# Windere/EAS-SNN

Measured on AMD Instinct MI355X. Metric: event-frames/sec (T=3) SYOLOX-S Gen1 304x240, higher is better.
Workload: dtype f32

## Files before the change

### eas_snn_amd/csrc/bn_lif.hip

```cpp
#include <stdlib.h>

#include <string.h>

#include "bn_lif_policy.h"
#include "eas_common.h"

namespace {

constexpr int VEC = 4;
constexpr int kMaxChunks = 64;
constexpr int NW = EAS_BLOCK / EAS_WAVE;

static inline int pick_chunks(int64_t groups_per_channel, int C) {
    int64_t want = (groups_per_channel + EAS_BLOCK - 1) / EAS_BLOCK;
    int64_t cap = 8192 / (C > 0 ? C : 1);
    if (cap < 1) cap = 1;
    if (cap > kMaxChunks) cap = kMaxChunks;
    if (want > cap) want = cap;
    if (want < 1) want = 1;
    return (int)want;
}

__global__ __launch_bounds__(EAS_BLOCK) void bn_stats_partial(const float* __restrict__ y, int TN, int C, int HW,
                                                              double* __restrict__ part, int Cy) {
// ... 4 lines not shown
    double s = 0.0, ss = 0.0;
    const int64_t stride = (int64_t)gridDim.x * blockDim.x;
    GroupWalk gw((int64_t)blockIdx.x * blockDim.x + threadIdx.x, stride, hw4);
    int64_t g = (int64_t)blockIdx.x * blockDim.x + threadIdx.x;
    for (; g + stride < groups; g += 2 * stride) {
        const float4 v0 = reinterpret_cast<const float4*>(y + (((int64_t)gw.n * Cy + c) * (int64_t)HW))[gw.q];
        gw.next();
        const float4 v1 = reinterpret_cast<const float4*>(y + (((int64_t)gw.n * Cy + c) * (int64_t)HW))[gw.q];
        gw.next();
        s += (double)v0.x + (double)v0.y + (double)v0.z + (double)v0.w;
        ss += (double)v0.x * v0.x + (double)v0.y * v0.y + (double)v0.z * v0.z + (double)v0.w * v0.w;
        s += (double)v1.x + (double)v1.y + (double)v1.z + (double)v1.w;
        ss += (double)v1.x * v1.x + (double)v1.y * v1.y + (double)v1.z * v1.z + (double)v1.w * v1.w;
    }
    if (g < groups) {
        const float4 v = reinterpret_cast<const float4*>(y + (((int64_t)gw.n * Cy + c) * (int64_t)HW))[gw.q];
        s += (double)v.x + (double)v.y + (double)v.z + (double)v.w;
        ss += (double)v.x * v.x + (double)v.y * v.y + (double)v.z * v.z + (double)v.w * v.w;
    }
    const double ts = eas_block_sum<double, NW>(s, red);
    const double tss = eas_block_sum<double, NW>(ss, red);
    if (threadIdx.x == 0) {
        part[((int64_t)c * kMaxChunks + blockIdx.x) * 2 + 0] = ts;
        part[((int64_t)c * kMaxChunks + blockIdx.x) * 2 + 1] = tss;
    }
}

__global__ __launch_bounds__(EAS_BLOCK) void bn_stats_partial_scalar(const float* __restrict__ y, int TN, int C, int HW,
                                                                     double* __restrict__ part) {
    __shared__ double red[NW];
    const int c = blockIdx.y;
    const int64_t groups = (int64_t)TN * HW;
    double s = 0.0, ss = 0.0;
    for (int64_t g = (int64_t)blockIdx.x * blockDim.x + threadIdx.x; g < groups; g += (int64_t)gridDim.x * blockDim.x) {
        const int64_t n = g / HW;
        const int q = (int)(g - n * HW);
        const float v = y[(n * C + c) * (int64_t)HW + q];
        s += v;
        ss += (double)v * v;
    }
    const double ts = eas_block_sum<double, NW>(s, red);
    const double tss = eas_block_sum<double, NW>(ss, red);
    if (threadIdx.x == 0) {
        part[((int64_t)c * kMaxChunks + blockIdx.x) * 2 + 0] = ts;
        part[((int64_t)c * kMaxChunks + blockIdx.x) * 2 + 1] = tss;
    }
}

__global__ __launch_bounds__(EAS_WAVE) void bn_stats_finalize(const double* __restrict__ part, int nchunks, double count,
                                                              int replicas, float eps, float momentum, float* __restrict__ mean,
                                                              float* __restrict__ invstd, float* __restrict__ rmean,
                                                              float* __restrict__ rvar) {
    const int c = blockIdx.x;
    double s = 0.0, ss = 0.0;
    if ((int)threadIdx.x < nchunks) {
        s = part[((int64_t)c * kMaxChunks + threadIdx.x) * 2 + 0];
        ss = part[((int64_t)c * kMaxChunks + threadIdx.x) * 2 + 1];
    }
    s = eas_wave_sum(s);
    ss = eas_wave_sum(ss);
    if (threadIdx.x == 0) {
        const double m = s / count;
        double var = ss / count - m * m;
        if (var < 0.0) var = 0.0;
        mean[c] = (float)m;
        invstd[c] = (float)(1.0 / sqrt(var + (double)eps));
        if (rmean) {
            const double full = count * replicas;
            const double unbiased = full > 1.0 ? var * full / (full - 1.0) : var;
            rmean[c] = (float)((1.0 - momentum) * rmean[c] + momentum * m);
            rvar[c] = (float)((1.0 - momentum) * rvar[c] + momentum * unbiased);
        }
    }
}

struct BnLifOut {
    const float* residual;
    int out_ctot;
    int y_ctot;
};

typedef __bf16 bf16x8 __attribute__((ext_vector_type(8)));

template <int T_, bool HARD, bool DI, bool STRICT>
__global__ __launch_bounds__(EAS_BLOCK) void bn_lif_fwd_kernel(const float* __restrict__ y, const float* __restrict__ mean,
                                                               const float* __restrict__ invstd,
                                                               const float* __restrict__ gamma,
                                                               const float* __restrict__ beta, const float* v_in, float* v_out,
                                                               EasLifParams p, float* __restrict__ spikes,
                                                               float* __restrict__ mean_out, int N, int C, int HW, int bcast,
                                                               BnFin fin, BnLifOut ox) {
    __shared__ float st[2];
    const int c = blockIdx.z * 8 + blockIdx.x;
    if (c >= C) return;
    const int chunk = blockIdx.y, nchunks_g = gridDim.y;
    float mu, istd;
    if (fin.part) {
        bn_finalize_in_block(fin, c, st, mu, istd, chunk == 0);
    } else {
        mu = mean[c];
        istd = invstd[c];
    }
    const float scale = gamma[c] * istd;
    const float shift = beta[c] - mu * scale;
    const int64_t Mo = ox.out_ctot ? (int64_t)N * ox.out_ctot * HW : (int64_t)N * C * HW;
    const float k = eas_lif_k(p);
    const float omk = 1.0f - k;
    const int hw4 = HW / VEC;
    const int64_t groups = (int64_t)N * hw4;
    const int64_t M = (int64_t)N * C * HW;
    const int Cy = ox.y_ctot ? ox.y_ctot : C;
    const int64_t yts = bcast ? 0 : (int64_t)N * Cy * HW;
    GroupWalk gw((int64_t)chunk * blockDim.x + threadIdx.x, (int64_t)nchunks_g * blockDim.x, hw4);
    for (int64_t g = (int64_t)chunk * blockDim.x + threadIdx.x; g < groups; g += (int64_t)nchunks_g * blockDim.x, gw.next()) {
        const int64_t n = gw.n;
        const int q = gw.q;
        const int64_t base = (n * C + c) * (int64_t)HW + (int64_t)q * VEC;
        float4 ys[T_];
        const int64_t ybase = (n * Cy + c) * (int64_t)HW + (int64_t)q * VEC;
#pragma unroll
        for (int t = 0; t < T_; ++t) ys[t] = *reinterpret_cast<const float4*>(y + (int64_t)t * yts + ybase);
        const float vr0 = HARD ? p.v_reset : 0.0f;
        float4 v = v_in ? *reinterpret_cast<const float4*>(v_in + base) : make_float4(vr0, vr0, vr0, vr0);
        float4 acc = make_float4(0.f, 0.f, 0.f, 0.f);
#pragma unroll
        for (int t = 0; t < T_; ++t) {
            float4 h, s;
            eas_lif_step<HARD, DI, STRICT>(v.x, fmaf(ys[t].x, scale, shift), k, omk, p.v_th, p.v_reset, h.x, s.x);
            eas_lif_step<HARD, DI, STRICT>(v.y, fmaf(ys[t].y, scale, shift), k, omk, p.v_th, p.v_reset, h.y, s.y);
            eas_lif_step<HARD, DI, STRICT>(v.z, fmaf(ys[t].z, scale, shift), k, omk, p.v_th, p.v_reset, h.z, s.z);
            eas_lif_step<HARD, DI, STRICT>(v.w, fmaf(ys[t].w, scale, shift), k, omk, p.v_th, p.v_reset, h.w, s.w);
            acc.x += s.x; acc.y += s.y; acc.z += s.z; acc.w += s.w;
            if (ox.residual) {
                const float4 r = *reinterpret_cast<const float4*>(ox.residual + (int64_t)t * M + base);
                s.x += r.x; s.y += r.y; s.z += r.z; s.w += r.w;
            }
            const int64_t obase = ox.out_ctot ? (n * ox.out_ctot + c) * (int64_t)HW + (int64_t)q * VEC : base;
            *reinterpret_cast<float4*>(spikes + (int64_t)t * Mo + obase) = s;
        }
        if (v_out) *reinterpret_cast<float4*>(v_out + base) = v;
        if (mean_out) {
            const float Tf = (float)T_;
            *reinterpret_cast<float4*>(mean_out + base) = make_float4(acc.x / Tf, acc.y / Tf, acc.z / Tf, acc.w / Tf);
        }
    }
}

__global__ __launch_bounds__(EAS_BLOCK) void bn_finalize_kernel(BnFin fin) {
    __shared__ float st[2];
    float mu, istd;
    bn_finalize_in_block(fin, (int)blockIdx.x, st, mu, istd, true);
}

template <int T_, bool HARD, bool DI, bool STRICT, int PV>
__global__ __launch_bounds__(EAS_BLOCK) void bn_lif_fwd_sp_kernel(const float* __restrict__ y, const float* __restrict__ mean,
                                                                  const float* __restrict__ invstd, const float* __restrict__ gamma,
                                                                  const float* __restrict__ beta, const float* v_in, float* v_out,
                                                                  EasLifParams p, bf16x8* __restrict__ planes, const bf16x8* __restrict__ res_planes,
                                                                  float* __restrict__ mean_out, int N, int C, int HW, int bcast, int y_ctot,
                                                                  int out_groups_tot, int res_groups_tot) {
    typedef float vecp __attribute__((ext_vector_type(PV)));
    const int grp = blockIdx.z * 8 + blockIdx.x;
    const int G = C / 8;
    if (grp >= G) return;
    const int chunk = blockIdx.y, nchunks_g = gridDim.y;
    float scale[8], shift[8];
#pragma unroll
    for (int j = 0; j < 8; ++j) {
        const int c = 8 * grp + j;
        scale[j] = gamma[c] * invstd[c];
        shift[j] = beta[c] - mean[c] * scale[j];
    }
    const float k = eas_lif_k(p);
    const float omk = 1.0f - k;
    const int hwp = HW / PV;
    const int64_t groups = (int64_t)N * hwp;
    const int Cy = y_ctot ? y_ctot : C;
    const int64_t yts = bcast ? 0 : (int64_t)N * Cy * HW;
    const float vr0 = HARD ? p.v_reset : 0.0f;
    const float Tf = (float)T_;
    GroupWalk gw((int64_t)chunk * blockDim.x + threadIdx.x, (int64_t)nchunks_g * blockDim.x, hwp);
    for (int64_t g = (int64_t)chunk * blockDim.x + threadIdx.x; g < groups; g += (int64_t)nchunks_g * blockDim.x, gw.next()) {
        const int64_t n = gw.n;
        const int q = gw.q;
        vecp ys[8][T_];
#pragma unroll
        for (int j = 0; j < 8; ++j) {
            const int64_t yb = (n * Cy + 8 * grp + j) * (int64_t)HW + (int64_t)q * PV;
#pragma unroll
            for (int t = 0; t < T_; ++t) ys[j][t] = *reinterpret_cast<const vecp*>(y + (int64_t)t * yts + yb);
        }
        float v[8][PV], acc[8][PV];
#pragma unroll
        for (int j = 0; j < 8; ++j) {
            vecp v0;
            if (v_in) v0 = *reinterpret_cast<const vecp*>(v_in + (n * C + 8 * grp + j) * (int64_t)HW + (int64_t)q * PV);
#pragma unroll
            for (int e = 0; e < PV; ++e) { v[j][e] = v_in ? v0[e] : vr0; acc[j][e] = 0.f; }
        }
#pragma unroll
        for (int t = 0; t < T_; ++t) {
            bf16x8 rp[PV];
            if (res_planes) {
#pragma unroll
                for (int e = 0; e < PV; ++e) rp[e] = res_planes[(((int64_t)t * N + n) * res_groups_tot + grp) * (int64_t)HW + (int64_t)q * PV + e];
            }
#pragma unroll
            for (int e = 0; e < PV; ++e) {
                bf16x8 o;
#pragma unroll
                for (int j = 0; j < 8; ++j) {
                    float h, s;
                    eas_lif_step<HARD, DI, STRICT>(v[j][e], fmaf(ys[j][t][e], scale[j], shift[j]), k, omk, p.v_th, p.v_reset, h, s);
                    acc[j][e] += s;
                    if (res_planes) s += (float)rp[e][j];
                    o[j] = (__bf16)s;
                }
                planes[(((int64_t)t * N + n) * out_groups_tot + grp) * (int64_t)HW + (int64_t)q * PV + e] = o;
            }
        }
#pragma unroll
        for (int j = 0; j < 8; ++j) {
            const int64_t base = (n * C + 8 * grp + j) * (int64_t)HW + (int64_t)q * PV;
            if (v_out) {
                vecp o;
#pragma unroll
                for (int e = 0; e < PV; ++e) o[e] = v[j][e];
                *reinterpret_cast<vecp*>(v_out + base) = o;
            }
            if (mean_out) {
                vecp o;
#pragma unroll
                for (int e = 0; e < PV; ++e) o[e] = acc[j][e] / Tf;
                *reinterpret_cast<vecp*>(mean_out + base) = o;
            }
        }
    }
}

template <int T_, bool HARD, bool DI, bool STRICT, class POL>
__device__ __forceinline__ void recompute_dz(const float (&yv)[T_], const float (&gs)[T_], float v0, float scale,
                                             float shift, float k, float omk, const EasLifParams& p, bool detach,
                                             int sg_id, float alpha, float (&dz)[T_], float& dk, float& da) {
    float h[T_], vprev[T_], z[T_];
    float v = v0;
#pragma unroll
    for (int t = 0; t < T_; ++t) {
        float s;
        vprev[t] = v;
        z[t] = fmaf(yv[t], scale, shift);
        eas_lif_step<HARD, DI, STRICT>(v, z[t], k, omk, p.v_th, p.v_reset, h[t], s);
    }
    float gv = 0.f;
#pragma unroll
    for (int t = T_ - 1; t >= 0; --t) {
        float dkt, gx;
        if constexpr (POL::fast)
            eas_lif_step_bwd_ct<HARD, DI, STRICT, POL::sg, POL::detach>(gs[t], gv, h[t], vprev[t], z[t], k, omk, p.v_th, p.v_reset, alpha, dkt,
                                                                        gx, da);
        else
            eas_lif_step_bwd<HARD, DI, STRICT>(gs[t], gv, h[t], vprev[t], z[t], k, omk, p.v_th, p.v_reset, detach, sg_id, alpha, dkt, gx, da);
        dz[t] = gx;
        dk += dkt;
    }
}

template <int T_, bool HARD, bool DI, bool STRICT, bool APPLY, class POL>
__global__ __launch_bounds__(EAS_BLOCK) void bn_lif_bwd_kernel(
    const float* __restrict__ grad_s, const float* __restrict__ grad_mean, const float* __restrict__ y,
    const float* __restrict__ mean, const float* __restrict__ invstd, const float* __restrict__ gamma,
    const float* __restrict__ beta, const float* __restrict__ v_init, EasLifParams p, int sg_id, float alpha,
    int batch_stats, double* __restrict__ part, int nchunks, float* __restrict__ grad_y, float* __restrict__ grad_gamma,
    float* __restrict__ grad_beta, float* __restrict__ grad_w, int N, int C, int HW, int bcast, int gs_ctot, int y_ctot,
    const float* __restrict__ alpha_dev, float* __restrict__ grad_alpha, int c_begin, int c_end, int finalize) {
    __shared__ double red[NW];
    __shared__ float bc[2];
    constexpr bool FAST = POL::fast;
    if (FAST) { bcast = 0; sg_id = POL::sg; }
    if (alpha_dev) alpha = fabsf(*alpha_dev);
    const int c = c_begin + blockIdx.z * 8 + blockIdx.x;
    if (c >= c_end) return;
    const int chunk = blockIdx.y, nchunks_g = gridDim.y;
    const float mu = mean[c], istd = invstd[c];
    const float scale = gamma[c] * istd;
    const float shift = beta[c] - mu * scale;
    const float k = eas_lif_k(p);
    const float omk = 1.0f - k;
    const bool detach = (p.flags & EAS_LIF_DETACH_RESET) != 0;
    const int hw4 = HW / VEC;
    const int64_t groups = (int64_t)N * hw4;
    const int64_t M = (int64_t)N * C * HW;
    const float invT = 1.0f / (float)T_;
    const int Cy = y_ctot ? y_ctot : C;
    const int64_t My = (int64_t)N * Cy * HW;
    const int64_t yts = bcast ? 0 : My;
    const int64_t Mg = gs_ctot ? (int64_t)N * gs_ctot * HW : M;
    const int Cg = gs_ctot ? gs_ctot : C;
    float m1 = 0.f, m2 = 0.f;
    if (APPLY) {
        if (threadIdx.x < EAS_WAVE) {
            double s1 = 0.0, s2 = 0.0;
            if ((int)threadIdx.x < nchunks) {
                s1 = part[((int64_t)c * kMaxChunks + threadIdx.x) * 4 + 0];
                s2 = part[((int64_t)c * kMaxChunks + threadIdx.x) * 4 + 1];
            }
            s1 = eas_wave_sum(s1);
            s2 = eas_wave_sum(s2);
            if (threadIdx.x == 0) {
                const double cnt = (double)T_ * N * HW;
                bc[0] = (float)(s1 / cnt);
                bc[1] = (float)(s2 / cnt);
                if (chunk == 0) {
                    grad_beta[c] = (float)s1;
                    grad_gamma[c] = (float)s2;
                }
            }
        }
        __syncthreads();
        if (batch_stats) { m1 = bc[0]; m2 = bc[1]; }
    }
    float s1 = 0.f, s2 = 0.f, dk = 0.f, da = 0.f;
    GroupWalk gw((int64_t)chunk * blockDim.x + threadIdx.x, (int64_t)nchunks_g * blockDim.x, hw4);
    for (int64_t g = (int64_t)chunk * blockDim.x + threadIdx.x; g < groups; g += (int64_t)nchunks_g * blockDim.x, gw.next()) {
        const int64_t n = gw.n;
        const int q = gw.q;
        const int64_t base = (n * C + c) * (int64_t)HW + (int64_t)q * VEC;
        float4 ys[T_], gsv[T_];
        const int64_t ybase = (n * Cy + c) * (int64_t)HW + (int64_t)q * VEC;
#pragma unroll
        for (int t = 0; t < T_; ++t) ys[t] = *reinterpret_cast<const float4*>(y + (int64_t)t * yts + ybase);
        float4 gm = make_float4(0.f, 0.f, 0.f, 0.f);
        if (!FAST && grad_mean) {
            gm = *reinterpret_cast<const float4*>(grad_mean + base);
            gm.x *= invT; gm.y *= invT; gm.z *= invT; gm.w *= invT;
        }
#pragma unroll
        for (int t = 0; t < T_; ++t) {
            gsv[t] = gm;
            if (FAST || grad_s) {
                const int64_t gbase = FAST ? (n * Cg + c) * (int64_t)HW + (int64_t)q * VEC
                                           : (gs_ctot ? (n * gs_ctot + c) * (int64_t)HW + (int64_t)q * VEC : base);
                const float4 g4 = *reinterpret_cast<const float4*>(grad_s + (int64_t)t * Mg + gbase);
                gsv[t].x += g4.x; gsv[t].y += g4.y; gsv[t].z += g4.z; gsv[t].w += g4.w;
            }
        }
        const float vr0 = HARD ? p.v_reset : 0.0f;
        float4 v0 = make_float4(vr0, vr0, vr0, vr0);
        if (!FAST && v_init) v0 = *reinterpret_cast<const float4*>(v_init + base);
        float4 outv[T_];
#pragma unroll
        for (int e = 0; e < VEC; ++e) {
            float yv[T_], gs[T_], dz[T_];
#pragma unroll
            for (int t = 0; t < T_; ++t) {
                yv[t] = reinterpret_cast<const float*>(&ys[t])[e];
                gs[t] = reinterpret_cast<const float*>(&gsv[t])[e];
            }
            const float v0e = reinterpret_cast<const float*>(&v0)[e];
            float dke = 0.f;
            recompute_dz<T_, HARD, DI, STRICT, POL>(yv, gs, v0e, scale, shift, k, omk, p, detach, sg_id, alpha, dz, dke, da);
#pragma unroll
            for (int t = 0; t < T_; ++t) {
                const float xhat = (yv[t] - mu) * istd;
                if (APPLY) {
                    reinterpret_cast<float*>(&outv[t])[e] = scale * (dz[t] - m1 - xhat * m2);
                } else {
                    s1 += dz[t];
                    s2 += dz[t] * xhat;
                }
            }
            dk += dke;
        }
        if (APPLY) {
            if (bcast) {
                float4 a = outv[0];
#pragma unroll
                for (int t = 1; t < T_; ++t) { a.x += outv[t].x; a.y += outv[t].y; a.z += outv[t].z; a.w += outv[t].w; }
                *reinterpret_cast<float4*>(grad_y + ybase) = a;
            } else {
#pragma unroll
                for (int t = 0; t < T_; ++t) *reinterpret_cast<float4*>(grad_y + (int64_t)t * My + ybase) = outv[t];
            }
        }
    }
    if (APPLY && grad_w && finalize && chunk == 0 && c == c_begin) {
        double acc = 0.0;
        for (int i = threadIdx.x; i < C * nchunks; i += blockDim.x) {
            const int cc = i / nchunks, j = i - cc * nchunks;
            acc += part[((int64_t)cc * kMaxChunks + j) * 4 + 2];
        }
        const double tot = eas_block_sum<double, NW>(acc, red);
        if (threadIdx.x == 0) *grad_w = (float)tot * (k * (1.0f - k));
    }
    if (APPLY && grad_alpha && finalize && chunk == 0 && c == c_begin) {
        double acc = 0.0;
        for (int i = threadIdx.x; i < C * nchunks; i += blockDim.x) {
            const int cc = i / nchunks, j = i - cc * nchunks;
            acc += part[((int64_t)cc * kMaxChunks + j) * 4 + 3];
        }
        const double tot = eas_block_sum<double, NW>(acc, red);
        if (threadIdx.x == 0) {
            const float a = *alpha_dev;
            *grad_alpha = (float)tot * (a > 0.f ? 1.f : (a < 0.f ? -1.f : 0.f));
        }
    }
    if (!APPLY) {
        const double t1 = eas_block_sum<double, NW>((double)s1, red);
        const double t2 = eas_block_sum<double, NW>((double)s2, red);
        const double t3 = eas_block_sum<double, NW>((double)dk, red);
        double t4 = 0.0;
        if (sg_id == EAS_SG_PATAN) t4 = eas_block_sum<double, NW>((double)da, red);
        if (threadIdx.x == 0) {
            double* o = part + ((int64_t)c * kMaxChunks + chunk) * 4;
            o[0] = t1; o[1] = t2; o[2] = t3; o[3] = t4;
        }
    }
}

template <int T_, bool HARD, bool DI, bool STRICT, int NT_, int GPT, class POL>
__global__ __launch_bounds__(NT_) void bn_lif_bwd_small_kernel(
    const float* __restrict__ grad_s, const float* __restrict__ grad_mean, const float* __restrict__ y,
    const float* __restrict__ mean, const float* __restrict__ invstd, const float* __restrict__ gamma,
    const float* __restrict__ beta, const float* __restrict__ v_init, EasLifParams p, int sg_id, float alpha,
    int batch_stats, double* __restrict__ part, float* __restrict__ grad_y, float* __restrict__ grad_gamma,
    float* __restrict__ grad_beta, int N, int C, int HW, int gs_ctot, int y_ctot, const float* __restrict__ alpha_dev) {
    constexpr int NWV = NT_ / EAS_WAVE;
    __shared__ double red[4][NWV];
    __shared__ float bc[2];
    if (POL::fast) sg_id = POL::sg;
    if (alpha_dev) alpha = fabsf(*alpha_dev);
    const int c = blockIdx.x;
    const float mu = mean[c], istd = invstd[c];
    const float scale = gamma[c] * istd;
    const float shift = beta[c] - mu * scale;
    const float k = eas_lif_k(p);
    const float omk = 1.0f - k;
    const bool detach = (p.flags & EAS_LIF_DETACH_RESET) != 0;
    const int hw4 = HW / VEC;
    const int groups = N * hw4;
    const int64_t M = (int64_t)N * C * HW;
    const int Cy = y_ctot ? y_ctot : C;
    const int64_t My = (int64_t)N * Cy * HW;
    const int64_t Mg = gs_ctot ? (int64_t)N * gs_ctot * HW : M;
    const float invT = 1.0f / (float)T_;
    float4 ys[GPT][T_], gsv[GPT][T_], v0[GPT];
    int64_t ybase[GPT];
#pragma unroll
    for (int i = 0; i < GPT; ++i) {
        const int g = threadIdx.x + i * NT_;
        const int gg = g < groups ? g : groups - 1;
        const int n = gg / hw4, q = gg - n * hw4;
        const int64_t base = ((int64_t)n * C + c) * (int64_t)HW + (int64_t)q * VEC;
        ybase[i] = ((int64_t)n * Cy + c) * (int64_t)HW + (int64_t)q * VEC;
#pragma unroll
        for (int t = 0; t < T_; ++t) ys[i][t] = *reinterpret_cast<const float4*>(y + (int64_t)t * My + ybase[i]);
        float4 gm = make_float4(0.f, 0.f, 0.f, 0.f);
        if (grad_mean) {
            gm = *reinterpret_cast<const float4*>(grad_mean + base);
            gm.x *= invT; gm.y *= invT; gm.z *= invT; gm.w *= invT;
        }
#pragma unroll
        for (int t = 0; t < T_; ++t) {
            gsv[i][t] = gm;
            if (grad_s) {
                const int64_t gbase = gs_ctot ? ((int64_t)n * gs_ctot + c) * (int64_t)HW + (int64_t)q * VEC : base;
                const float4 g4 = *reinterpret_cast<const float4*>(grad_s + (int64_t)t * Mg + gbase);
                gsv[i][t].x += g4.x; gsv[i][t].y += g4.y; gsv[i][t].z += g4.z; gsv[i][t].w += g4.w;
            }
        }
        const float vr0 = HARD ? p.v_reset : 0.0f;
        v0[i] = make_float4(vr0, vr0, vr0, vr0);
        if (v_init) v0[i] = *reinterpret_cast<const float4*>(v_init + base);
    }
    float s1 = 0.f, s2 = 0.f, dk = 0.f, da = 0.f;
#pragma unroll
    for (int i = 0; i < GPT; ++i) {
        const bool live = threadIdx.x + i * NT_ < groups;
#pragma unroll
        for (int e = 0; e < VEC; ++e) {
            float yv[T_], gs[T_], dz[T_];
#pragma unroll
            for (int t = 0; t < T_; ++t) {
                yv[t] = reinterpret_cast<const float*>(&ys[i][t])[e];
                gs[t] = reinterpret_cast<const float*>(&gsv[i][t])[e];
            }
            float dke = 0.f, dae = 0.f;
            recompute_dz<T_, HARD, DI, STRICT, POL>(yv, gs, reinterpret_cast<const float*>(&v0[i])[e], scale, shift, k, omk, p, detach, sg_id, alpha, dz, dke, dae);
            if (live) {
#pragma unroll
                for (int t = 0; t < T_; ++t) {
                    s1 += dz[t];
                    s2 += dz[t] * ((yv[t] - mu) * istd);
                }
                dk += dke;
                da += dae;
            }
        }
    }
    double t1 = eas_wave_sum((double)s1), t2 = eas_wave_sum((double)s2), t3 = eas_wave_sum((double)dk), t4 = eas_wave_sum((double)da);
    if ((threadIdx.x & (EAS_WAVE - 1)) == 0) {
        const int w = threadIdx.x / EAS_WAVE;
        red[0][w] = t1; red[1][w] = t2; red[2][w] = t3; red[3][w] = t4;
    }
    __syncthreads();
    if (threadIdx.x == 0) {
        t1 = t2 = t3 = t4 = 0.0;
        for (int w = 0; w < NWV; ++w) { t1 += red[0][w]; t2 += red[1][w]; t3 += red[2][w]; t4 += red[3][w]; }
        const double cnt = (double)T_ * N * HW;
        bc[0] = (float)(t1 / cnt);
        bc[1] = (float)(t2 / cnt);
        grad_beta[c] = (float)t1;
        grad_gamma[c] = (float)t2;
        double* o = part + ((int64_t)c * kMaxChunks) * 4;
        o[0] = t1; o[1] = t2; o[2] = t3; o[3] = sg_id == EAS_SG_PATAN ? t4 : 0.0;
    }
    __syncthreads();
    const float m1 = batch_stats ? bc[0] : 0.f, m2 = batch_stats ? bc[1] : 0.f;
#pragma unroll
    for (int i = 0; i < GPT; ++i) {
        if (threadIdx.x + i * NT_ >= groups) continue;
        float4 outv[T_];
#pragma unroll
        for (int e = 0; e < VEC; ++e) {
            float yv[T_], gs[T_], dz[T_];
#pragma unroll
            for (int t = 0; t < T_; ++t) {
                yv[t] = reinterpret_cast<const float*>(&ys[i][t])[e];
                gs[t] = reinterpret_cast<const float*>(&gsv[i][t])[e];
            }
            float dke = 0.f, dae = 0.f;
            recompute_dz<T_, HARD, DI, STRICT, POL>(yv, gs, reinterpret_cast<const float*>(&v0[i])[e], scale, shift, k, omk, p, detach, sg_id, alpha, dz, dke, dae);
#pragma unroll
            for (int t = 0; t < T_; ++t) reinterpret_cast<float*>(&outv[t])[e] = scale * (dz[t] - m1 - ((yv[t] - mu) * istd) * m2);
        }
#pragma unroll
        for (int t = 0; t < T_; ++t) *reinterpret_cast<float4*>(grad_y + (int64_t)t * My + ybase[i]) = outv[t];
    }
}

__global__ __launch_bounds__(EAS_BLOCK) void bn_lif_bwd_scalars_kernel(const double* __restrict__ part, int C, EasLifParams p, float* __restrict__ grad_w,
                                                                       const float* __restrict__ alpha_dev, float* __restrict__ grad_alpha) {
    __shared__ double red[NW];
    const float k = eas_lif_k(p);
    if (grad_w) {
        double acc = 0.0;
        for (int i = threadIdx.x; i < C; i += blockDim.x) acc += part[((int64_t)i * kMaxChunks) * 4 + 2];
        const double tot = eas_block_sum<double, NW>(acc, red);
        if (threadIdx.x == 0) *grad_w = (float)tot * (k * (1.0f - k));
    }
    if (grad_alpha) {
        double acc = 0.0;
        for (int i = threadIdx.x; i < C; i += blockDim.x) acc += part[((int64_t)i * kMaxChunks) * 4 + 3];
        const double tot = eas_block_sum<double, NW>(acc, red);
        if (threadIdx.x == 0) {
            const float a = *alpha_dev;
            *grad_alpha = (float)tot * (a > 0.f ? 1.f : (a < 0.f ? -1.f : 0.f));
        }
    }
}

template <int T_, bool HARD, bool DI, bool STRICT>
int launch_fwd_t(const float* y, const float* mean, const float* invstd, const float* gamma, const float* beta,
                 const float* v_in, float* v_out, EasLifParams p, float* spikes, float* mean_out, int N, int C, int HW,
                 int bcast, const BnFin& fin, const BnLifOut& ox, bf16x8* planes, const bf16x8* res_planes, int out_groups, int res_groups,
                 hipStream_t st) {
    if (planes) {
        if (fin.part) {
            EAS_LAUNCH(bn_finalize_kernel, dim3(C), dim3(EAS_BLOCK), 0, st, fin);
            EAS_CHECK_LAUNCH();
        }
        constexpr int PV = 1;
        const int chunks = pick_chunks((int64_t)N * (HW / PV), C / 8);
        EAS_LAUNCH((bn_lif_fwd_sp_kernel<T_, HARD, DI, STRICT, PV>), EAS_CHAN_GRID(chunks, C / 8), dim3(EAS_BLOCK), 0, st, y,
                           mean, invstd, gamma, beta, v_in,
                           v_out, p, planes, res_planes, mean_out, N, C, HW, bcast, ox.y_ctot, out_groups, res_groups);
        EAS_CHECK_LAUNCH();
        return EAS_OK;
    }
    const int chunks = pick_chunks((int64_t)N * (HW / VEC), C);
    EAS_LAUNCH((bn_lif_fwd_kernel<T_, HARD, DI, STRICT>), EAS_CHAN_GRID(chunks, C), dim3(EAS_BLOCK), 0, st, y, mean,
                       invstd, gamma, beta, v_in, v_out, p, spikes, mean_out, N, C, HW, bcast, fin, ox);
    EAS_CHECK_LAUNCH();
    return EAS_OK;
}

template <bool HARD, bool DI, bool STRICT>
int launch_fwd(int T, const float* y, const float* mean, const float* invstd, const float* gamma, const float* beta,
               const float* v_in, float* v_out, EasLifParams p, float* spikes, float* mean_out, int N, int C, int HW,
               int bcast, const BnFin& fin, const BnLifOut& ox, bf16x8* planes, const bf16x8* res_planes, int out_groups, int res_groups,
               hipStream_t st) {
#define EAS_CASE(TT) \
    case TT: return launch_fwd_t<TT, HARD, DI, STRICT>(y, mean, invstd, gamma, beta, v_in, v_out, p, spikes, mean_out, N, C, HW, bcast, fin, ox, planes, res_planes, out_groups, res_groups, st);
    switch (T) {
        EAS_CASE(1) EAS_CASE(2) EAS_CASE(3) EAS_CASE(4) EAS_CASE(5) EAS_CASE(6) EAS_CASE(7) EAS_CASE(8)
        default: return EAS_ERR_UNSUPPORTED;
    }
#undef EAS_CASE
}

struct BwdCall {
    const float *grad_s, *grad_mean, *y, *mean, *invstd, *gamma, *beta, *v_init;
    EasLifParams p;
    int sg;
    float alpha;
    int batch_stats;
    float *grad_y, *grad_gamma, *grad_beta, *grad_w;
    double* ws;
    int T, N, C, HW, bcast, gs_ctot, y_ctot;
    const float* alpha_dev;
    float* grad_alpha;
    hipStream_t st;
};

static inline bool bwd_form(const char* word) {
    const char* form = getenv("EAS_BNLIF_BWD");
    return form && strstr(form, word);
}

static inline int bwd_one_pass_gpt(const BwdCall& c) {
    const int gpt = c.T <= 3 ? 3 : (c.T <= 5 ? 2 : 1);
    const int64_t groups = (int64_t)c.N * (c.HW / VEC);
    return (!bwd_form("two") && !c.bcast && c.C >= 64 && groups <= 512 * gpt) ? gpt : 0;
}

template <int T_, bool HARD, bool DI, bool STRICT, class POL>
int launch_bwd_t(const BwdCall& c) {
    const int N = c.N, C = c.C, HW = c.HW;
    const int chunks = pick_chunks((int64_t)N * (HW / VEC), C);
    if (bwd_one_pass_gpt(c)) {
        constexpr int GPT = T_ <= 3 ? 3 : (T_ <= 5 ? 2 : 1);
        const int64_t groups = (int64_t)N * (HW / VEC);
#define EAS_SMALL(NT_) EAS_LAUNCH((bn_lif_bwd_small_kernel<T_, HARD, DI, STRICT, NT_, GPT, POL>), dim3(C), dim3(NT_), 0, c.st, c.grad_s, c.grad_mean, c.y, \
                                   c.mean, c.invstd, c.gamma, c.beta, c.v_init, c.p, c.sg, c.alpha, c.batch_stats, c.ws, c.grad_y, c.grad_gamma,       \
                                   c.grad_beta, N, C, HW, c.gs_ctot, c.y_ctot, c.alpha_dev)
        if (groups <= 256 * GPT) EAS_SMALL(256);
        else EAS_SMALL(512);
#undef EAS_SMALL
        EAS_CHECK_LAUNCH();
        if (c.grad_w || c.grad_alpha) {
            EAS_LAUNCH(bn_lif_bwd_scalars_kernel, dim3(1), dim3(EAS_BLOCK), 0, c.st, c.ws, C, c.p, c.grad_w, c.alpha_dev, c.grad_alpha);
            EAS_CHECK_LAUNCH();
        }
        return EAS_OK;
    }
    static const int group_mb = eas_dev_env("EAS_BNLIF_BWD_GROUP_MB") ? atoi(eas_dev_env("EAS_BNLIF_BWD_GROUP_MB")) : 0;
    int gc = C;
    if (group_mb > 0) {
        const double per_channel = (double)N * HW * 4.0 * ((c.bcast ? 1 : T_) + T_);
        gc = (int)(group_mb * 1048576.0 / per_channel) / 8 * 8;
        if (gc < 8) gc = 8;
        if (gc > C) gc = C;
    }
    for (int c0 = 0; c0 < C; c0 += gc) {
        const int c1 = c0 + gc < C ? c0 + gc : C;
        const int last = c1 == C;
        EAS_LAUNCH((bn_lif_bwd_kernel<T_, HARD, DI, STRICT, false, POL>), EAS_CHAN_GRID(chunks, c1 - c0), dim3(EAS_BLOCK), 0, c.st, c.grad_s,
                   c.grad_mean, c.y, c.mean, c.invstd, c.gamma, c.beta, c.v_init, c.p, c.sg, c.alpha, c.batch_stats, c.ws, chunks, c.grad_y,
                   c.grad_gamma, c.grad_beta, (float*)nullptr, N, C, HW, c.bcast, c.gs_ctot, c.y_ctot, c.alpha_dev, (float*)nullptr, c0, c1, 0);
        EAS_CHECK_LAUNCH();
        EAS_LAUNCH((bn_lif_bwd_kernel<T_, HARD, DI, STRICT, true, POL>), EAS_CHAN_GRID(chunks, c1 - c0), dim3(EAS_BLOCK), 0, c.st, c.grad_s,
                   c.grad_mean, c.y, c.mean, c.invstd, c.gamma, c.beta, c.v_init, c.p, c.sg, c.alpha, c.batch_stats, c.ws, chunks, c.grad_y,
                   c.grad_gamma, c.grad_beta, c.grad_w, N, C, HW, c.bcast, c.gs_ctot, c.y_ctot, c.alpha_dev, c.grad_alpha, c0, c1, last);
        EAS_CHECK_LAUNCH();
    }
    return EAS_OK;
}

struct BwdRow {
    int T;
    bool hard, di;
    int sg;
    bool detach;
    int (*fn)(const BwdCall&);
};
template <int T_, bool HARD, bool DI, int SG = EAS_SG_RUNTIME, bool DETACH = false>
constexpr BwdRow bwd_row() {
    return {T_, HARD, DI, SG, DETACH, launch_bwd_t<T_, HARD, DI, false, BnLifBwdPolicy<SG, DETACH>>};
}
#define EAS_BWD_GENERIC_ROWS(H, D) \
    bwd_row<1, H, D>(), bwd_row<2, H, D>(), bwd_row<3, H, D>(), bwd_row<4, H, D>(), bwd_row<5, H, D>(), bwd_row<6, H, D>(), bwd_row<7, H, D>(), bwd_row<8, H, D>()
const BwdRow kBwdInstances[] = {
    bwd_row<3, false, false, EAS_SG_ATAN>(), bwd_row<5, false, false, EAS_SG_ATAN>(), bwd_row<7, false, false, EAS_SG_ATAN>(),
    EAS_BWD_GENERIC_ROWS(false, false), EAS_BWD_GENERIC_ROWS(true, false), EAS_BWD_GENERIC_ROWS(false, true), EAS_BWD_GENERIC_ROWS(true, true),
};
#undef EAS_BWD_GENERIC_ROWS

int bwd_select(const BwdCall& c) {
    const bool hard = c.p.flags & EAS_LIF_HARD_RESET, di = c.p.flags & EAS_LIF_DECAY_INPUT, detach = c.p.flags & EAS_LIF_DETACH_RESET;
    if (c.p.flags & EAS_LIF_FIRE_STRICT) return EAS_ERR_UNSUPPORTED;
    const bool plain = bwd_one_pass_gpt(c) || (c.grad_s && !c.grad_mean && !c.v_init && !c.bcast);
    const bool fast_ok = plain && !bwd_form("generic");
    for (const BwdRow& r : kBwdInstances) {
        if (r.T != c.T || r.hard != hard || r.di != di) continue;
        if (r.sg == EAS_SG_RUNTIME || (fast_ok && r.sg == c.sg && r.detach == detach)) return r.fn(c);
    }
    return EAS_ERR_UNSUPPORTED;
}

}

extern "C" {

int64_t eas_bn_workspace_doubles(int C) { return (int64_t)C * kMaxChunks * 4; }

static int stats_partial(const float* y, int TN, int C, int HW, double* workspace, int y_ctot, hipStream_t st) {
    const int Cy = y_ctot ? y_ctot : C;
    int chunks;
    if (HW % VEC == 0 && (((uintptr_t)y) & 15) == 0) {
        chunks = pick_chunks((int64_t)TN * (HW / VEC), C);
        EAS_LAUNCH(bn_stats_partial, dim3(chunks, C), dim3(EAS_BLOCK), 0, st, y, TN, C, HW, workspace, Cy);
    } else {
        if (Cy != C) return EAS_ERR_UNSUPPORTED;
        chunks = pick_chunks((int64_t)TN * HW, C);
        EAS_LAUNCH(bn_stats_partial_scalar, dim3(chunks, C), dim3(EAS_BLOCK), 0, st, y, TN, C, HW, workspace);
    }
    if (hipGetLastError() != hipSuccess) return EAS_ERR_LAUNCH;
    return chunks;
}

int eas_bn_stats(const float* y, int TN, int C, int HW, int replicas, float eps, float momentum, float* mean,
                 float* invstd, float* running_mean, float* running_var, double* workspace, eas_stream_t stream) {
    if (!y || !mean || !invstd || !workspace || TN < 1 || C < 1 || HW < 1 || replicas < 1) return EAS_ERR_INVALID_ARG;
    if ((running_mean == nullptr) != (running_var == nullptr)) return EAS_ERR_INVALID_ARG;
    if (C > 65535) return EAS_ERR_UNSUPPORTED;
    hipStream_t st = eas_s(stream);
    EAS_CLEAR_ERR();
    const int chunks = stats_partial(y, TN, C, HW, workspace, 0, st);
    if (chunks < 0) return chunks;
// ... 126 lines not shown
```

### eas_snn_amd/csrc/eas_common.h

```cpp
#pragma once
#include <hip/hip_runtime.h>
#include <stdint.h>
#include <stdlib.h>

#include "../../include/eas_hip.h"

#define EAS_WAVE 64
#define EAS_BLOCK 256

#define EAS_CLEAR_ERR() (void)hipGetLastError()
#define EAS_CHECK_LAUNCH()                                          \
    do {                                                            \
        if (hipGetLastError() != hipSuccess) return EAS_ERR_LAUNCH; \
    } while (0)

static inline hipStream_t eas_s(eas_stream_t s) { return reinterpret_cast<hipStream_t>(s); }

__attribute__((visibility("hidden"))) extern int eas_trace_on;
__attribute__((visibility("hidden"))) extern long long eas_launch_count;
__attribute__((visibility("hidden"))) void eas_trace_kernel(const void* host_function);
#define EAS_LAUNCH(kern, ...)                                                \
    do {                                                                     \
        auto eas_kern_ = (kern);                                             \
        ++eas_launch_count;                                                  \
// ... 17 lines not shown
__device__ __forceinline__ float eas_sigmoidf(float x) { return 1.0f / (1.0f + __expf(-x)); }

__device__ __forceinline__ float eas_surrogate_grad(int id, float alpha, float u) {
    if (id == EAS_SG_ATAN || id == EAS_SG_PATAN) {
        const float q = 1.57079632679489661923f * alpha * u;
        return alpha * 0.5f * __builtin_amdgcn_rcpf(1.0f + q * q);
    } else if (id == EAS_SG_SIGMOID) {
        const float sg = eas_sigmoidf(alpha * u);
        return (1.0f - sg) * sg * alpha;
    } else {
        return (fabsf(u) < 0.5f / alpha) ? alpha : 0.0f;
    }
}

template <typename T>
__device__ __forceinline__ T eas_wave_sum(T v) {
#pragma unroll
    for (int off = EAS_WAVE / 2; off > 0; off >>= 1) v += __shfl_down(v, off, EAS_WAVE);
    return v;
}

template <typename T, int NW>
__device__ __forceinline__ T eas_block_sum(T v, T* smem) {
    const int lane = threadIdx.x & (EAS_WAVE - 1);
    const int wid = threadIdx.x / EAS_WAVE;
    v = eas_wave_sum(v);
    if (lane == 0) smem[wid] = v;
    __syncthreads();
    T r = T(0);
    if (threadIdx.x == 0) {
#pragma unroll
        for (int i = 0; i < NW; ++i) r += smem[i];
    }
    __syncthreads();
    return r;
}

template <int CTRL, int ROW_MASK>
__device__ __forceinline__ float eas_dpp(float v) {
    return __builtin_bit_cast(float, __builtin_amdgcn_update_dpp(0, __builtin_bit_cast(int, v), CTRL, ROW_MASK, 0xF, false));
}
__device__ __forceinline__ float eas_half_wave_sum(float v) {
    v += eas_dpp<0xB1, 0xF>(v);
    v += eas_dpp<0x4E, 0xF>(v);
    v += eas_dpp<0x141, 0xF>(v);
    v += eas_dpp<0x140, 0xF>(v);
    v += eas_dpp<0x142, 0xA>(v);
    return v;
}

#define EAS_STATS_PITCH 36
#define EAS_STATS_SCRATCH (32 * EAS_STATS_PITCH)
template <int WM, int WN, typename ACC>
__device__ __forceinline__ void eas_conv_stats_wave(const ACC (&acc)[WM][WN], const bool (&valid)[WN], float* scratch, double* red, int lane) {
    typedef float f2 __attribute__((ext_vector_type(2)));
    const int h = lane >> 5, r = lane & 31;
    bool all = true;
#pragma unroll
    for (int n = 0; n < WN; ++n) all = all && valid[n];
    const bool uniform_all = __all(all);
#pragma unroll
    for (int m = 0; m < WM; ++m) {
        f2 s[8], q[8];
#pragma unroll
        for (int p = 0; p < 8; ++p) { s[p] = f2{0.0f, 0.0f}; q[p] = f2{0.0f, 0.0f}; }
        if (uniform_all) {
#pragma unroll
            for (int n = 0; n < WN; ++n)
#pragma unroll
                for (int p = 0; p < 8; ++p) {
                    const f2 a = f2{acc[m][n][2 * p], acc[m][n][2 * p + 1]};
                    s[p] += a;
                    q[p] = __builtin_elementwise_fma(a, a, q[p]);
                }
        } else {
#pragma unroll
            for (int n = 0; n < WN; ++n)
#pragma unroll
                for (int p = 0; p < 8; ++p) {
                    const f2 a = f2{valid[n] ? acc[m][n][2 * p] : 0.0f, valid[n] ? acc[m][n][2 * p + 1] : 0.0f};
                    s[p] += a;
                    q[p] = __builtin_elementwise_fma(a, a, q[p]);
                }
        }
#pragma unroll
        for (int stat = 0; stat < 2; ++stat) {
#pragma unroll
            for (int e = 0; e < 16; ++e) {
                const f2 v = stat ? q[e >> 1] : s[e >> 1];
                scratch[(4 * h + (e & 3) + 8 * (e >> 2)) * EAS_STATS_PITCH + r] = (e & 1) ? v.y : v.x;
            }
            __builtin_amdgcn_fence(__ATOMIC_RELEASE, "wavefront");
            __builtin_amdgcn_wave_barrier();
            __builtin_amdgcn_fence(__ATOMIC_ACQUIRE, "wavefront");
            if (lane < 32) {
                const float4* row = reinterpret_cast<const float4*>(scratch + lane * EAS_STATS_PITCH);
                double t = 0.0;
#pragma unroll
                for (int k = 0; k < 8; ++k) {
                    const float4 v = row[k];
                    t += (double)v.x; t += (double)v.y; t += (double)v.z; t += (double)v.w;
                }
                red[(m * 32 + lane) * 2 + stat] = t;
            }
            __builtin_amdgcn_fence(__ATOMIC_RELEASE, "wavefront");
            __builtin_amdgcn_wave_barrier();
            __builtin_amdgcn_fence(__ATOMIC_ACQUIRE, "wavefront");
        }
    }
}

__device__ __forceinline__ void eas_conv_stats_store(const double* red, int wave_stride, int nwv, int t, int co, int Cout, double* stats, int nb,
                                                     int block) {
    if (co >= Cout) return;
    double s = 0.0, q = 0.0;
    for (int w = 0; w < nwv; ++w) {
        s += red[w * wave_stride + t * 2 + 0];
        q += red[w * wave_stride + t * 2 + 1];
    }
    *reinterpret_cast<double2*>(stats + ((int64_t)co * nb + block) * 2) = make_double2(s, q);
}

#define EAS_BN_MAX_CHUNKS 64

struct BnFin {
    const double* part;
    int nchunks, pitch, replicas;
    double count;
    float eps, momentum;
    float* mean_out;
    float* invstd_out;
    float* rmean;
    float* rvar;
};

__device__ __forceinline__ void bn_from_totals(const BnFin& f, int c, double s, double ss, bool publish, float& mu, float& istd) {
    const double m = s / f.count;
    double var = ss / f.count - m * m;
    if (var < 0.0) var = 0.0;
    mu = (float)m;
    istd = (float)(1.0 / sqrt(var + (double)f.eps));
    if (publish) {
        f.mean_out[c] = mu;
        f.invstd_out[c] = istd;
        if (f.rmean) {
            const double full = f.count * f.replicas;
            const double unbiased = full > 1.0 ? var * full / (full - 1.0) : var;
            f.rmean[c] = (float)((1.0 - f.momentum) * f.rmean[c] + f.momentum * m);
            f.rvar[c] = (float)((1.0 - f.momentum) * f.rvar[c] + f.momentum * unbiased);
        }
    }
}

__device__ __forceinline__ void bn_finalize_in_block(const BnFin& f, int c, float* st, float& mu, float& istd, bool publish) {
    if (f.nchunks > EAS_WAVE) {
        __shared__ double fred[2][EAS_BLOCK / EAS_WAVE];
        const double2* p = reinterpret_cast<const double2*>(f.part) + (int64_t)c * f.pitch;
        const int B = blockDim.x, n = f.nchunks;
        double s = 0.0, ss = 0.0;
        for (int i = threadIdx.x; i < n; i += 4 * B) {
            const double2 z = make_double2(0.0, 0.0);
            const double2 v0 = p[i];
            const double2 v1 = i + B < n ? p[i + B] : z;
            const double2 v2 = i + 2 * B < n ? p[i + 2 * B] : z;
            const double2 v3 = i + 3 * B < n ? p[i + 3 * B] : z;
            s += v0.x; ss += v0.y;
            s += v1.x; ss += v1.y;
            s += v2.x; ss += v2.y;
            s += v3.x; ss += v3.y;
        }
        s = eas_wave_sum(s);
        ss = eas_wave_sum(ss);
        if ((threadIdx.x & (EAS_WAVE - 1)) == 0) {
            fred[0][threadIdx.x / EAS_WAVE] = s;
            fred[1][threadIdx.x / EAS_WAVE] = ss;
        }
        __syncthreads();
        if (threadIdx.x == 0) {
            s = 0.0; ss = 0.0;
            for (int w = 0; w < (int)(blockDim.x / EAS_WAVE); ++w) { s += fred[0][w]; ss += fred[1][w]; }
            float m_, i_;
            bn_from_totals(f, c, s, ss, publish, m_, i_);
            st[0] = m_;
            st[1] = i_;
        }
        __syncthreads();
        mu = st[0];
        istd = st[1];
        return;
    }
    if (threadIdx.x < EAS_WAVE) {
        double s = 0.0, ss = 0.0;
        if ((int)threadIdx.x < f.nchunks) {
            s = f.part[((int64_t)c * f.pitch + threadIdx.x) * 2 + 0];
            ss = f.part[((int64_t)c * f.pitch + threadIdx.x) * 2 + 1];
        }
        s = eas_wave_sum(s);
        ss = eas_wave_sum(ss);
        if (threadIdx.x == 0) {
            const double m = s / f.count;
            double var = ss / f.count - m * m;
            if (var < 0.0) var = 0.0;
            st[0] = (float)m;
            st[1] = (float)(1.0 / sqrt(var + (double)f.eps));
            if (publish) {
                f.mean_out[c] = st[0];
                f.invstd_out[c] = st[1];
                if (f.rmean) {
                    const double full = f.count * f.replicas;
                    const double unbiased = full > 1.0 ? var * full / (full - 1.0) : var;
                    f.rmean[c] = (float)((1.0 - f.momentum) * f.rmean[c] + f.momentum * m);
                    f.rvar[c] = (float)((1.0 - f.momentum) * f.rvar[c] + f.momentum * unbiased);
                }
            }
        }
    }
    __syncthreads();
    mu = st[0];
    istd = st[1];
}

#define EAS_CHAN_GRID(chunks, C) dim3(8, (chunks), ((C) + 7) / 8)

struct GroupWalk {
    int n, q, dn, dq, hw4;
    __device__ __forceinline__ GroupWalk(int64_t g0, int64_t stride, int hw4_) : hw4(hw4_) {
        n = (int)(g0 / hw4_);
        q = (int)(g0 - (int64_t)n * hw4_);
        dn = (int)(stride / hw4_);
        dq = (int)(stride - (int64_t)dn * hw4_);
    }
    __device__ __forceinline__ void next() {
        n += dn;
        q += dq;
        if (q >= hw4) {
            q -= hw4;
            ++n;
        }
    }
};

struct EasLifParams {
    const float* w_logit;
    float k_const;
    float v_th;
    float v_reset;
    int flags;
};

__device__ __forceinline__ float eas_lif_k(const EasLifParams& p) {
    return p.w_logit ? eas_sigmoidf(*p.w_logit) : p.k_const;
}

template <bool HARD, bool DI, bool STRICT>
__device__ __forceinline__ void eas_lif_step(float& v, float x, float k, float omk, float v_th, float v_reset,
                                             float& h, float& s) {
    if (DI) {
        h = HARD ? v + (x - (v - v_reset)) * k : v + (x - v) * k;
    } else {
        h = (HARD && v_reset != 0.0f) ? (v - (v - v_reset) * k) + x : v * omk + x;
    }
    const float u = h - v_th;
    s = STRICT ? (u > 0.0f ? 1.0f : 0.0f) : (u >= 0.0f ? 1.0f : 0.0f);
    v = HARD ? (1.0f - s) * h + s * v_reset : h - s * v_th;
}

template <bool HARD, bool DI, bool STRICT>
__device__ __forceinline__ float eas_lif_step_bwd(float gs, float& gv, float h, float v_prev, float x, float k,
                                                  float omk, float v_th, float v_reset, bool detach, int sg_id,
                                                  float alpha, float& dk_term, float& gx, float& da) {
    const float u = h - v_th;
    const float s = STRICT ? (u > 0.0f ? 1.0f : 0.0f) : (u >= 0.0f ? 1.0f : 0.0f);
    const float sg = eas_surrogate_grad(sg_id, alpha, u);
    if (sg_id == EAS_SG_PATAN) {
        const float q = 1.57079632679489661923f * alpha * u;
        const float gs_all = detach ? gs : (HARD ? gs + gv * (v_reset - h) : gs - gv * v_th);
        da += gs_all * (0.5f * u * __builtin_amdgcn_rcpf(1.0f + q * q));
    }
    float dvdh;
    if (HARD) {
        dvdh = detach ? (1.0f - s) : (1.0f - s) + (v_reset - h) * sg;
    } else {
        dvdh = detach ? 1.0f : 1.0f - v_th * sg;
    }
    const float dh = gs * sg + gv * dvdh;
    if (DI) {
        gx = dh * k;
        dk_term = dh * (HARD ? (x - (v_prev - v_reset)) : (x - v_prev));
    } else {
        gx = dh;
        dk_term = dh * ((HARD && v_reset != 0.0f) ? -(v_prev - v_reset) : -v_prev);
    }
    gv = dh * omk;
    return dh;
}
```

Baseline: 3417.

## Fold BN finalize into spike-plane forward kernel and prefetch y across iterations

The forward BN+LIF spike-plane path now finalizes batch statistics inside each block for its 8 channels, which removes the separate bn_finalize launch when the partial-sum buffer is small enough. It also issues the first y loads before the finalize reduction and prefetches the next iteration's y during the loop to hide latency. Every chunk block redundantly reduces the partials, and only chunk 0 publishes the results. The shared finalize helper is generalized to NC channels, and a waves-per-EU occupancy hint is added to the small backward kernel.

Measured after the change: 3409. About the same (-0.3%).

```diff
diff --git a/eas_snn_amd/csrc/bn_lif.hip b/eas_snn_amd/csrc/bn_lif.hip
--- a/eas_snn_amd/csrc/bn_lif.hip
+++ b/eas_snn_amd/csrc/bn_lif.hip
@@ -180,44 +180,40 @@
     bn_finalize_in_block(fin, (int)blockIdx.x, st, mu, istd, true);
 }
 
-template <int T_, bool HARD, bool DI, bool STRICT, int PV>
+constexpr int kFoldDepth = 1;
+template <int T_, bool HARD, bool DI, bool STRICT, int PV, bool FOLD>
 __global__ __launch_bounds__(EAS_BLOCK) void bn_lif_fwd_sp_kernel(const float* __restrict__ y, const float* __restrict__ mean,
                                                                   const float* __restrict__ invstd, const float* __restrict__ gamma,
                                                                   const float* __restrict__ beta, const float* v_in, float* v_out,
                                                                   EasLifParams p, bf16x8* __restrict__ planes, const bf16x8* __restrict__ res_planes,
                                                                   float* __restrict__ mean_out, int N, int C, int HW, int bcast, int y_ctot,
-                                                                  int out_groups_tot, int res_groups_tot) {
+                                                                  int out_groups_tot, int res_groups_tot, BnFin fin) {
     typedef float vecp __attribute__((ext_vector_type(PV)));
+    __shared__ float st[8][2];
     const int grp = blockIdx.z * 8 + blockIdx.x;
     const int G = C / 8;
     if (grp >= G) return;
     const int chunk = blockIdx.y, nchunks_g = gridDim.y;
-    float scale[8], shift[8];
-#pragma unroll
-    for (int j = 0; j < 8; ++j) {
-        const int c = 8 * grp + j;
-        scale[j] = gamma[c] * invstd[c];
-        shift[j] = beta[c] - mean[c] * scale[j];
-    }
-    const float k = eas_lif_k(p);
-    const float omk = 1.0f - k;
     const int hwp = HW / PV;
     const int64_t groups = (int64_t)N * hwp;
     const int Cy = y_ctot ? y_ctot : C;
     const int64_t yts = bcast ? 0 : (int64_t)N * Cy * HW;
+    const int64_t stride = (int64_t)nchunks_g * blockDim.x;
+    GroupWalk gw((int64_t)chunk * blockDim.x + threadIdx.x, stride, hwp);
+    auto load_y = [&](vecp (&ys)[8][T_]) {
+#pragma unroll
+        for (int j = 0; j < 8; ++j) {
+            const int64_t yb = ((int64_t)gw.n * Cy + 8 * grp + j) * (int64_t)HW + (int64_t)gw.q * PV;
+#pragma unroll
+            for (int t = 0; t < T_; ++t) ys[j][t] = *reinterpret_cast<const vecp*>(y + (int64_t)t * yts + yb);
+        }
+    };
+    float scale[8], shift[8];
+    const float k = eas_lif_k(p);
+    const float omk = 1.0f - k;
     const float vr0 = HARD ? p.v_reset : 0.0f;
     const float Tf = (float)T_;
-    GroupWalk gw((int64_t)chunk * blockDim.x + threadIdx.x, (int64_t)nchunks_g * blockDim.x, hwp);
-    for (int64_t g = (int64_t)chunk * blockDim.x + threadIdx.x; g < groups; g += (int64_t)nchunks_g * blockDim.x, gw.next()) {
-        const int64_t n = gw.n;
-        const int q = gw.q;
-        vecp ys[8][T_];
-#pragma unroll
-        for (int j = 0; j < 8; ++j) {
-            const int64_t yb = (n * Cy + 8 * grp + j) * (int64_t)HW + (int64_t)q * PV;
-#pragma unroll
-            for (int t = 0; t < T_; ++t) ys[j][t] = *reinterpret_cast<const vecp*>(y + (int64_t)t * yts + yb);
-        }
+    auto neuron = [&](const vecp (&ys)[8][T_], const int64_t n, const int q) {
         float v[8][PV], acc[8][PV];
 #pragma unroll
         for (int j = 0; j < 8; ++j) {
@@ -262,6 +258,39 @@
                 for (int e = 0; e < PV; ++e) o[e] = acc[j][e] / Tf;
                 *reinterpret_cast<vecp*>(mean_out + base) = o;
             }
+        }
+    };
+    if constexpr (FOLD) {
+        int64_t g = (int64_t)chunk * blockDim.x + threadIdx.x;
+        vecp ys[8][T_];
+        if (g < groups) load_y(ys);
+        float mu[8], istd[8];
+        bn_finalize_in_block_nc<8, kFoldDepth>(fin, 8 * grp, st, mu, istd, chunk == 0);
+#pragma unroll
+        for (int j = 0; j < 8; ++j) {
+            const int c = 8 * grp + j;
+            scale[j] = gamma[c] * istd[j];
+            shift[j] = beta[c] - mu[j] * scale[j];
+        }
+        while (g < groups) {
+            const int64_t n = gw.n;
+            const int q = gw.q;
+            neuron(ys, n, q);
+            g += stride;
+            gw.next();
+            if (g < groups) load_y(ys);
+        }
+    } else {
+#pragma unroll
+        for (int j = 0; j < 8; ++j) {
+            const int c = 8 * grp + j;
+            scale[j] = gamma[c] * invstd[c];
+            shift[j] = beta[c] - mean[c] * scale[j];
+        }
+        for (int64_t g = (int64_t)chunk * blockDim.x + threadIdx.x; g < groups; g += stride, gw.next()) {
+            vecp ys[8][T_];
+            load_y(ys);
+            neuron(ys, gw.n, gw.q);
         }
     }
 }
@@ -445,8 +474,10 @@
     }
 }
 
+constexpr int bwd_small_waves(int t, int nt, bool fast) { return nt == 512 ? (fast && t <= 3 ? 4 : 2) : 1; }
+
 template <int T_, bool HARD, bool DI, bool STRICT, int NT_, int GPT, class POL>
-__global__ __launch_bounds__(NT_) void bn_lif_bwd_small_kernel(
+__global__ __launch_bounds__(NT_) __attribute__((amdgpu_waves_per_eu(bwd_small_waves(T_, NT_, POL::fast)))) void bn_lif_bwd_small_kernel(
     const float* __restrict__ grad_s, const float* __restrict__ grad_mean, const float* __restrict__ y,
     const float* __restrict__ mean, const float* __restrict__ invstd, const float* __restrict__ gamma,
     const float* __restrict__ beta, const float* __restrict__ v_init, EasLifParams p, int sg_id, float alpha,
@@ -587,21 +618,34 @@
     }
 }
 
+constexpr int64_t kFwdFoldMaxBytes = 4 << 20;
+static inline bool fwd_fold(int chunks, int channel_groups, int nchunks) {
+    const char* form = getenv("EAS_BNLIF_FWD");
+    if (form && strstr(form, "separate")) return false;
+    if (form && strstr(form, "fold")) return true;
+    return (int64_t)chunks * channel_groups * 8 * nchunks * 16 <= kFwdFoldMaxBytes;
+}
+
 template <int T_, bool HARD, bool DI, bool STRICT>
 int launch_fwd_t(const float* y, const float* mean, const float* invstd, const float* gamma, const float* beta,
                  const float* v_in, float* v_out, EasLifParams p, float* spikes, float* mean_out, int N, int C, int HW,
                  int bcast, const BnFin& fin, const BnLifOut& ox, bf16x8* planes, const bf16x8* res_planes, int out_groups, int res_groups,
                  hipStream_t st) {
     if (planes) {
-        if (fin.part) {
-            EAS_LAUNCH(bn_finalize_kernel, dim3(C), dim3(EAS_BLOCK), 0, st, fin);
-            EAS_CHECK_LAUNCH();
-        }
         constexpr int PV = 1;
         const int chunks = pick_chunks((int64_t)N * (HW / PV), C / 8);
-        EAS_LAUNCH((bn_lif_fwd_sp_kernel<T_, HARD, DI, STRICT, PV>), EAS_CHAN_GRID(chunks, C / 8), dim3(EAS_BLOCK), 0, st, y,
-                           mean, invstd, gamma, beta, v_in,
-                           v_out, p, planes, res_planes, mean_out, N, C, HW, bcast, ox.y_ctot, out_groups, res_groups);
+#define EAS_SP(FOLD_) EAS_LAUNCH((bn_lif_fwd_sp_kernel<T_, HARD, DI, STRICT, PV, FOLD_>), EAS_CHAN_GRID(chunks, C / 8), dim3(EAS_BLOCK), 0, st, y, \
+                                 mean, invstd, gamma, beta, v_in, v_out, p, planes, res_planes, mean_out, N, C, HW, bcast, ox.y_ctot, out_groups, res_groups, fin)
+        if (fin.part && fwd_fold(chunks, C / 8, fin.nchunks)) {
+            EAS_SP(true);
+        } else {
+            if (fin.part) {
+                EAS_LAUNCH(bn_finalize_kernel, dim3(C), dim3(EAS_BLOCK), 0, st, fin);
+                EAS_CHECK_LAUNCH();
+            }
+            EAS_SP(false);
+        }
+#undef EAS_SP
         EAS_CHECK_LAUNCH();
         return EAS_OK;
     }
diff --git a/eas_snn_amd/csrc/eas_common.h b/eas_snn_amd/csrc/eas_common.h
--- a/eas_snn_amd/csrc/eas_common.h
+++ b/eas_snn_amd/csrc/eas_common.h
@@ -193,72 +193,93 @@
     }
 }
 
+template <int NC, int D>
+__device__ __forceinline__ void bn_finalize_in_block_nc(const BnFin& f, int c0, float (*st)[2], float (&mu)[NC], float (&istd)[NC], bool publish) {
+    if (f.nchunks > EAS_WAVE) {
+        __shared__ double fred[NC][2][EAS_BLOCK / EAS_WAVE];
+        const double2* p = reinterpret_cast<const double2*>(f.part) + (int64_t)c0 * f.pitch;
+        const int B = blockDim.x, n = f.nchunks;
+        double s[NC], ss[NC];
+#pragma unroll
+        for (int j = 0; j < NC; ++j) { s[j] = 0.0; ss[j] = 0.0; }
+        for (int i = threadIdx.x; i < n; i += D * B) {
+            const double2 z = make_double2(0.0, 0.0);
+            double2 v[NC][D];
+#pragma unroll
+            for (int j = 0; j < NC; ++j) {
+                const double2* pj = p + (int64_t)j * f.pitch;
+#pragma unroll
+                for (int d = 0; d < D; ++d) v[j][d] = i + d * B < n ? pj[i + d * B] : z;
+            }
+#pragma unroll
+            for (int j = 0; j < NC; ++j) {
+#pragma unroll
+                for (int d = 0; d < D; ++d) { s[j] += v[j][d].x; ss[j] += v[j][d].y; }
+            }
+        }
+#pragma unroll
+        for (int j = 0; j < NC; ++j) {
+            s[j] = eas_wave_sum(s[j]);
+            ss[j] = eas_wave_sum(ss[j]);
+        }
+        if ((threadIdx.x & (EAS_WAVE - 1)) == 0) {
+#pragma unroll
+            for (int j = 0; j < NC; ++j) {
+                fred[j][0][threadIdx.x / EAS_WAVE] = s[j];
+                fred[j][1][threadIdx.x / EAS_WAVE] = ss[j];
+            }
+        }
+        __syncthreads();
+        if (threadIdx.x < NC) {
+            const int j = threadIdx.x;
+            double ts = 0.0, tss = 0.0;
+            for (int w = 0; w < (int)(blockDim.x / EAS_WAVE); ++w) { ts += fred[j][0][w]; tss += fred[j][1][w]; }
+            float m_, i_;
+            bn_from_totals(f, c0 + j, ts, tss, publish, m_, i_);
+            st[j][0] = m_;
+            st[j][1] = i_;
+        }
+    } else if (threadIdx.x < EAS_WAVE) {
+        double s[NC], ss[NC];
+#pragma unroll
+        for (int j = 0; j < NC; ++j) {
+            s[j] = 0.0; ss[j] = 0.0;
+            if ((int)threadIdx.x < f.nchunks) {
+                s[j] = f.part[((int64_t)(c0 + j) * f.pitch + threadIdx.x) * 2 + 0];
+                ss[j] = f.part[((int64_t)(c0 + j) * f.pitch + threadIdx.x) * 2 + 1];
+            }
+        }
+#pragma unroll
+        for (int j = 0; j < NC; ++j) {
+            s[j] = eas_wave_sum(s[j]);
+            ss[j] = eas_wave_sum(ss[j]);
+        }
+        double ts = s[0], tss = ss[0];
+#pragma unroll
+        for (int j = 1; j < NC; ++j) {
+            const double a = __shfl(s[j], 0, EAS_WAVE), b = __shfl(ss[j], 0, EAS_WAVE);
+            if ((int)threadIdx.x == j) { ts = a; tss = b; }
+        }
+        if (threadIdx.x < NC) {
+            float m_, i_;
+            bn_from_totals(f, c0 + (int)threadIdx.x, ts, tss, publish, m_, i_);
+            st[threadIdx.x][0] = m_;
+            st[threadIdx.x][1] = i_;
+        }
+    }
+    __syncthreads();
+#pragma unroll
+    for (int j = 0; j < NC; ++j) {
+        mu[j] = st[j][0];
+        istd[j] = st[j][1];
+    }
+}
+
 __device__ __forceinline__ void bn_finalize_in_block(const BnFin& f, int c, float* st, float& mu, float& istd, bool publish) {
-    if (f.nchunks > EAS_WAVE) {
-        __shared__ double fred[2][EAS_BLOCK / EAS_WAVE];
-        const double2* p = reinterpret_cast<const double2*>(f.part) + (int64_t)c * f.pitch;
-        const int B = blockDim.x, n = f.nchunks;
-        double s = 0.0, ss = 0.0;
-        for (int i = threadIdx.x; i < n; i += 4 * B) {
-            const double2 z = make_double2(0.0, 0.0);
-            const double2 v0 = p[i];
-            const double2 v1 = i + B < n ? p[i + B] : z;
-            const double2 v2 = i + 2 * B < n ? p[i + 2 * B] : z;
-            const double2 v3 = i + 3 * B < n ? p[i + 3 * B] : z;
-            s += v0.x; ss += v0.y;
-            s += v1.x; ss += v1.y;
-            s += v2.x; ss += v2.y;
-            s += v3.x; ss += v3.y;
-        }
-        s = eas_wave_sum(s);
-        ss = eas_wave_sum(ss);
-        if ((threadIdx.x & (EAS_WAVE - 1)) == 0) {
-            fred[0][threadIdx.x / EAS_WAVE] = s;
-            fred[1][threadIdx.x / EAS_WAVE] = ss;
-        }
-        __syncthreads();
-        if (threadIdx.x == 0) {
-            s = 0.0; ss = 0.0;
-            for (int w = 0; w < (int)(blockDim.x / EAS_WAVE); ++w) { s += fred[0][w]; ss += fred[1][w]; }
-            float m_, i_;
-            bn_from_totals(f, c, s, ss, publish, m_, i_);
-            st[0] = m_;
-            st[1] = i_;
-        }
-        __syncthreads();
-        mu = st[0];
-        istd = st[1];
-        return;
-    }
-    if (threadIdx.x < EAS_WAVE) {
-        double s = 0.0, ss = 0.0;
-        if ((int)threadIdx.x < f.nchunks) {
-            s = f.part[((int64_t)c * f.pitch + threadIdx.x) * 2 + 0];
-            ss = f.part[((int64_t)c * f.pitch + threadIdx.x) * 2 + 1];
-        }
-        s = eas_wave_sum(s);
-        ss = eas_wave_sum(ss);
-        if (threadIdx.x == 0) {
-            const double m = s / f.count;
-            double var = ss / f.count - m * m;
-            if (var < 0.0) var = 0.0;
-            st[0] = (float)m;
-            st[1] = (float)(1.0 / sqrt(var + (double)f.eps));
-            if (publish) {
-                f.mean_out[c] = st[0];
-                f.invstd_out[c] = st[1];
-                if (f.rmean) {
-                    const double full = f.count * f.replicas;
-                    const double unbiased = full > 1.0 ? var * full / (full - 1.0) : var;
-                    f.rmean[c] = (float)((1.0 - f.momentum) * f.rmean[c] + f.momentum * m);
-                    f.rvar[c] = (float)((1.0 - f.momentum) * f.rvar[c] + f.momentum * unbiased);
-                }
-            }
-        }
-    }
-    __syncthreads();
-    mu = st[0];
-    istd = st[1];
+    float m_[1], i_[1];
+    bn_finalize_in_block_nc<1, 4>(f, c, reinterpret_cast<float (*)[2]>(st), m_, i_, publish);
+    mu = m_[0];
+    istd = i_[0];
 }
 
 #define EAS_CHAN_GRID(chunks, C) dim3(8, (chunks), ((C) + 7) / 8)
```
